# schmeing/ReSeq

Measured on AMD Instinct MI355X. Metric: simulated read-pairs/sec (2x150 bp), higher is better.
Workload: dtype f64

## Files before the change

### reseq_amd/csrc/rsq_host.cpp

```cpp
#include <stdio.h>
#include "rsq_host.h"
#include "rsq_textio.h"

#include <errno.h>
#include <fcntl.h>
#include <string.h>
#include <sys/mman.h>
#include <sys/stat.h>
#include <unistd.h>
#include <zlib.h>

#include <algorithm>
#include <array>
#include <atomic>
#include <chrono>
#include <exception>
#include <memory>
#include <mutex>

#include <fstream>
#include <thread>

#include "rsq_core.h"

namespace rsq {

Options &options() {
    static Options o;
    return o;
}
namespace {
struct OptionEntry {
    const char *name;
    int64_t Options::*field;
};
const OptionEntry kOptionTable[] = {
    {"fill_mode", &Options::fill_mode},         {"image_tiles", &Options::image_tiles},     {"rate_rows", &Options::rate_rows},
    {"no_indel_skip", &Options::no_indel_skip}, {"force_exact", &Options::force_exact},     {"base_call_word", &Options::base_call_word},     {"min_quality_quads", &Options::min_quality_quads},
    {"trace_plan", &Options::trace_plan},       {"trace_prepare", &Options::trace_prepare},
    {"bias_window", &Options::bias_window},     {"window_chunks", &Options::window_chunks}, {"serial_fasta", &Options::serial_fasta},   {"trace_load", &Options::trace_load},
    {"chain_chunk", &Options::chain_chunk},     {"chain_warmup", &Options::chain_warmup},
    {"serial_parse", &Options::serial_parse},   {"parse_stretch", &Options::parse_stretch}, {"mapped_parses", &Options::mapped_parses},
    {"fasta_stretch", &Options::fasta_stretch}, {"overlap", &Options::overlap}, {"specialize", &Options::specialize}, {"job_write_direct", &Options::job_write_direct},             {"job_chunk_bytes", &Options::job_chunk_bytes}, {"host_gzip", &Options::host_gzip}, {"fill_waves", &Options::fill_waves}, {"fasta_no_stage", &Options::fasta_no_stage},
    {"hiprtc_by_name", &Options::hiprtc_by_name}, {"gzip_route", &Options::gzip_route},       {"gzip_stretch", &Options::gzip_stretch},
    {"sieve_lds", &Options::sieve_lds},         {"sieve_lds_bytes", &Options::sieve_lds_bytes}, {"sieve_tracks_mb", &Options::sieve_tracks_mb},
    {"wide_rows", &Options::wide_rows},
    {"stats_chunk", &Options::stats_chunk},     {"stats_slab", &Options::stats_slab},       {"stats_groups", &Options::stats_groups},   {"stats_form", &Options::stats_form},
};
}
bool set_option(const char *name, int64_t value) {
    for (const OptionEntry &e : kOptionTable)
        if (0 == strcmp(name, e.name)) {
            options().*(e.field) = value;
            return true;
        }
    return false;
}
bool get_option(const char *name, int64_t *value) {
    for (const OptionEntry &e : kOptionTable)
        if (0 == strcmp(name, e.name)) {
            *value = options().*(e.field);
            return true;
        }
    return false;
}
const char *option_names() {
    static const std::string names = [] {
        std::string s;
        for (const OptionEntry &e : kOptionTable) s += (s.empty() ? "" : " ") + std::string(e.name);
        return s;
    }();
    return names.c_str();
}

static size_t pad8(size_t n) { return (8 - (n & 7)) & 7; }

Container::Container(const std::string &path) {
    std::ifstream f(path, std::ios::binary | std::ios::ate);
    if (!f) throw Error("cannot open profile '" + path + "'");
    std::streamsize sz = f.tellg();
    f.seekg(0);
    buf_.resize((size_t)sz);
    if (!f.read(reinterpret_cast<char *>(buf_.data()), sz)) throw Error("cannot read profile '" + path + "'");
    if (buf_.size() < 16 || memcmp(buf_.data(), "RSQPROF1", 8) != 0) throw Error("'" + path + "' is not an RSQP profile container");
    uint32_t version, n;
    memcpy(&version, &buf_[8], 4);
    memcpy(&n, &buf_[12], 4);
    if (version != 1) throw Error("unsupported RSQP version");
    static const size_t kSize[7] = {1, 2, 4, 8, 4, 8, 8};
    size_t pos = 16;
    for (uint32_t i = 0; i < n; ++i) {
        if (pos + 4 > buf_.size()) throw Error("truncated RSQP container");
        uint16_t ln;
        memcpy(&ln, &buf_[pos], 2);
        std::string name(reinterpret_cast<const char *>(&buf_[pos + 2]), ln);
        Array a;
        a.dtype = buf_[pos + 2 + ln];
        int ndim = buf_[pos + 3 + ln];
// ... 1206 lines not shown
```

### reseq_amd/csrc/rsq_host.h

```cpp
#pragma once
#include <stdint.h>

#include <map>
#include <stdexcept>
#include <string>
#include <string.h>
#include <vector>

namespace rsq {

struct Error : std::runtime_error {
    using std::runtime_error::runtime_error;
};

struct Options {
    int64_t fill_mode = -1;
    int64_t image_tiles = 0;
    int64_t rate_rows = 0;
    int64_t no_indel_skip = 0;
    int64_t base_call_word = 1;
    int64_t force_exact = 0;
    int64_t min_quality_quads = 0;
    int64_t trace_plan = 0;
    int64_t trace_prepare = 0;
    int64_t bias_window = 0;
    int64_t window_chunks = 0;
    int64_t trace_load = 0;
    int64_t serial_fasta = 0;
    int64_t fasta_stretch = 0;
    int64_t chain_chunk = 0;
    int64_t chain_warmup = -1;
    int64_t serial_parse = 0;
    int64_t mapped_parses = 0;
    int64_t parse_stretch = 0;
    int64_t job_chunk_bytes = 0;
    int64_t job_write_direct = 0;
    int64_t specialize = 1;
    int64_t fasta_no_stage = 0;
    int64_t fill_waves = 0;
    int64_t host_gzip = 0;
    int64_t gzip_route = -1;
    int64_t gzip_stretch = 0;
    int64_t hiprtc_by_name = 0;
    int64_t sieve_lds = 1;
    int64_t sieve_lds_bytes = 0;
    int64_t sieve_tracks_mb = 4096;
    int64_t wide_rows = 0;
    int64_t overlap = 0;
    int64_t stats_chunk = 0;
    int64_t stats_slab = 0;
    int64_t stats_groups = 0;
    int64_t stats_form = 0;
};
Options &options();
bool set_option(const char *name, int64_t value);
bool get_option(const char *name, int64_t *value);
const char *option_names();

struct Array {
    int dtype = 0;
    std::vector<uint64_t> dims;
    uint64_t count = 0;
    const uint8_t *data = nullptr;
};

class Container {
   public:
    explicit Container(const std::string &path);
    const Array &get(const std::string &name) const;
    bool has(const std::string &name) const { return arrays_.count(name) != 0; }
    template <class T>
    std::vector<T> vec(const std::string &name, int dtype) const {
        const Array &a = get(name);
        if (a.dtype != dtype) throw Error("profile array '" + name + "' has the wrong type");
        const T *p = reinterpret_cast<const T *>(a.data);
        return std::vector<T>(p, p + a.count);
    }
    template <class T>
    T scalar(const std::string &name, int dtype) const {
        return vec<T>(name, dtype).at(0);
    }

   private:
    std::vector<uint8_t> buf_;
    std::map<std::string, Array> arrays_;
};

template <class T>
struct Vect {
    uint64_t from = 0;
    std::vector<T> v;
    uint64_t to() const { return from + v.size(); }
    T operator[](uint64_t i) const { return (i < from || i >= to()) ? T(0) : v[i - from]; }
};

struct HostTable {
    uint32_t nm = 0;
    std::vector<uint32_t> par0;
    uint32_t from[4] = {0, 0, 0, 0}, to[4] = {0, 0, 0, 0};
// ... 139 lines not shown
```

### reseq_amd/csrc/rsq_sieve.h

```cpp
#pragma once
#include "rsq_core.h"
#include "rsq_variants.h"

namespace rsq {

struct SieveSite {
    uint32_t seq, start, L;
    uint64_t word_off;
    const double *thr;
    uint32_t group;
    uint32_t sur_start[3];
    bool have_start;
    uint32_t sub;
    VarStart st;
};

RSQ_HD uint32_t site_c1(const SieveSite &site) { return site.seq | (site.sub << 22); }

struct GapTables {
    const double *q_;
    const uint32_t *seg_end_;
    const double *thr_;
    RSQ_HD double q(uint32_t len) const { return q_[len]; }
    RSQ_HD uint32_t seg_end(uint32_t len) const { return seg_end_[len]; }
    RSQ_HD double thr1(uint32_t len) const { return thr_[2u * len + 1u]; }
};
RSQ_HD GapTables gap_tables(const DevSim &S, const SieveSite &site) {
    return GapTables{S.gap_q + (size_t)site.group * S.insert_to, S.gap_seg_end + (size_t)site.group * S.insert_to, site.thr};
}
template <class T, class F>
RSQ_HD uint32_t sieve_gaps_in(const DevSim &S, const SieveSite &site, const T &tab, F &&on_pass) {
    const uint32_t c1 = site_c1(site);
    uint32_t cur = S.insert_from, k = 0, n = 0;
    while (cur < S.insert_to) {
        const Words w = philox(S.seed, site.start, c1, k++, kDomSieve << 28);
        const uint32_t e = tab.seg_end(cur);
        const double base = (cur == S.insert_from || tab.seg_end(cur - 1u) == cur) ? 1.0 : tab.q(cur - 1u);
        const double target = u53_to_unit(w.w0, w.w1) * base;
        uint32_t lo = cur, hi = e;
        while (lo < hi) {
            const uint32_t mid = (lo + hi) >> 1;
            if (tab.q(mid) <= target) hi = mid;
            else lo = mid + 1u;
        }
        if (lo < e) {
            const double thr1 = tab.thr1(lo);
            on_pass(lo, thr1 + u53_to_unit(w.w2, w.w3) * (1 - thr1));
            ++n;
            cur = lo + 1u;
        } else cur = e;
    }
    return n;
}
template <class F>
// ... 461 lines not shown
        if (at < hit_cap) hits[at] = h;
        intra += (uint32_t)h.cnt0 + h.cnt1;
    }
    if (c < cand_cap) pairs_of[c] = n_here;
}

template <int VM>
__global__ void __launch_bounds__(256) k_sieve_emit(DevSim S, uint32_t block_lo, uint32_t block_hi, const SieveHit *hits, uint32_t n_hits, const uint64_t *cand_off,
                                                   const uint64_t *pair_off, Fragment *frags, FragmentVar *fvars, const SlotInfo *slots, const SieveCand *cands = nullptr,
                                                   const uint32_t *pairs_of = nullptr, const uint32_t *cell_info = nullptr) {
    const uint32_t i = blockIdx.x * blockDim.x + threadIdx.x;
    if (i >= n_hits) return;
    SieveHit h;
    if constexpr (VM == 0) {
        const uint32_t pairs = pairs_of[i];
        if (!pairs) return;
        const SieveCand cand = cands[i];
        const uint32_t info = cell_info[i];
        h.slot = cand.slot;
        h.cand = i;
        h.intra = 0;
        h.len = (uint16_t)cand.len;
        h.cnt0 = (uint16_t)(info & 0xFFFFu);
        h.cnt1 = (uint16_t)(pairs - (info & 0xFFFFu));
        h.strand0 = (uint8_t)((info >> 16) & 1u);
        h.strand1 = (uint8_t)((info >> 17) & 1u);
        h.allele0 = h.allele1 = 0;
    } else h = hits[i];
    SieveSite site;
    uint32_t first_slot;
    const uint32_t block_id = init_site_slot<VM>(S, block_lo, block_hi, h.slot, site, &first_slot, slots);
    const uint64_t base = pair_off[h.cand];
    const uint32_t number_base = (uint32_t)(base - pair_off[cand_off[first_slot]]);
    uint32_t k = h.intra;
    for (uint32_t e = 0; e < 2u; ++e) {
        const uint32_t cnt = e ? h.cnt1 : h.cnt0, strand = e ? h.strand1 : h.strand0, allele = e ? h.allele1 : h.allele0;
        if (!cnt) continue;
        FragmentVar fv{};
        if constexpr (VM == 2) {
            const AlleleCell ac = allele_cell(allele_view(S, site.seq, allele), site.st, site.start, h.len);
            fv.end = ac.end;
            fv.sub = site.sub;
            fv.start_var = site.st.first_variant_id;
            fv.start_var_pos = site.st.start_variant_pos;
            fv.end_var = ac.end_var.first_variant_id;
            fv.end_var_pos = ac.end_var.start_variant_pos;
        }
        for (uint32_t dup = 0; dup < cnt; ++dup, ++k) {
            frags[base + k] = make_fragment(site, h.len, dup, strand, block_id, number_base + k + 1u, allele);
            if constexpr (VM == 2) fvars[base + k] = fv;
        }
    }
}
#endif

}
```

### reseq_amd/csrc/rsq_sim.hip

```cpp
#include <hip/hip_runtime.h>
#include <fcntl.h>
#include <sys/mman.h>
#include <sys/stat.h>
#include <math.h>
#include <string.h>
#include <unistd.h>

#include <algorithm>
#include <atomic>
#include <chrono>
#include <map>
#include <thread>
#include <type_traits>
#include <memory>
#include <string>
#include <utility>
#include <vector>

#include "../../include/reseq_amd.h"
#include "rsq_deflate.h"
#include "rsq_fasta.h"
#include "rsq_chains.h"
#include "rsq_sieve.h"
#include "rsq_scan.h"
// ... 143 lines not shown
        std::vector<std::unique_ptr<DevBuf>> &own = owned[current_scope];
        own.emplace_back(new DevBuf());
        own.back()->reserve(bytes + 8);
        HIP_CHECK(hipMemcpy(own.back()->as<void>(), data, bytes, hipMemcpyHostToDevice));
        return own.back()->as<void>();
    }
    void *put_zeros(size_t bytes) override {
        std::vector<std::unique_ptr<DevBuf>> &own = owned[current_scope];
        own.emplace_back(new DevBuf());
        own.back()->reserve(bytes + 8);
        HIP_CHECK(hipMemset(own.back()->as<void>(), 0, bytes + 8));
        return own.back()->as<void>();
    }
    void write_bytes(void *dst, const void *src, size_t bytes) override { HIP_CHECK(hipMemcpy(dst, src, bytes, hipMemcpyHostToDevice)); }
    void read_bytes(void *dst_host, const void *src, size_t bytes) override { HIP_CHECK(hipMemcpy(dst_host, src, bytes, hipMemcpyDeviceToHost)); }
};

struct MappedFile {
    const char *data = nullptr;
    size_t size = 0;
    explicit MappedFile(const char *path) {
        const int fd = open(path, O_RDONLY);
        if (fd < 0) throw Error(std::string("cannot open ") + path + ": " + strerror(errno));
        struct stat st;
        if (fstat(fd, &st) != 0 || st.st_size <= 0) {
            close(fd);
            throw Error(std::string(path) + " is empty or cannot be examined");
        }
        size = (size_t)st.st_size;
        void *p = mmap(nullptr, size, PROT_READ, MAP_PRIVATE, fd, 0);
        close(fd);
        if (p == MAP_FAILED) throw Error(std::string("cannot map ") + path);
        data = static_cast<const char *>(p);
    }
    ~MappedFile() {
        if (data) munmap(const_cast<char *>(data), size);
    }
    MappedFile(const MappedFile &) = delete;
    MappedFile &operator=(const MappedFile &) = delete;
};

struct rsq_sim : PrepassSim {
    int device = 0;
    DeviceUploader up;
    struct Workspace {
        DevBuf fvars;
        DevBuf slot_table;
        DevBuf counts, offsets, tile_sums, scan_total, frags, raw_seq, raw_qual, raw_ops, raw_meta, sizes, off_r1, off_r2, fill_counters, hits, hit_count, cands, pairs_of, pair_off, templates, rec_flags, rec_index, rec_count;
        DevBuf bin_keys, bin_small, bin_perm, bin_frags, bin_fvars;
        DevBuf fa_counts, fa_first, fa_at, fa_len, fa_id_len, fa_frag_len, fa_seg, fa_codes, fa_summary;
        DevBuf sam_sizes, sam_side, off_sam;
        DevBuf bam_side;
        DevBuf cell_info;
        hipEvent_t text_done = nullptr;
    } ws[2];
    struct JobText {
        std::vector<std::unique_ptr<DevBuf>> chunks[2];
        std::vector<size_t> used[2];
        uint64_t bytes[2] = {0, 0};
        bool complete = false;
        std::vector<unsigned char> packed[2];
        bool is_packed = false;
        bool device_packed = false;
        void clear() {
            complete = false;
            is_packed = false;
            device_packed = false;
            for (auto &p : packed) std::vector<unsigned char>().swap(p);
            for (int f = 0; f < 2; ++f) {
                chunks[f].clear();
                used[f].clear();
                bytes[f] = 0;
            }
        }
    } job;
    DevBuf totals;
    bool gz_dense = false;
    bool gz_keep_code = false, gz_have_code = false;
    DevBuf gz_slots, gz_sizes, gz_at, gz_hist, gz_codes, gz_total;
    Workspace *cur = &ws[0];
    hipStream_t side[2] = {nullptr, nullptr};
    hipEvent_t ev_call = nullptr, ev_fill = nullptr, ev_emit = nullptr;
    std::map<std::string, Timer> timers;
    uint32_t n_cu = 256;
    struct Mailbox {
        struct Sieve {
            uint64_t total, n_cands;
            uint32_t n_hits;
        } sieve[2];
        uint64_t r1_bytes, r2_bytes, truth_bytes;
        uint32_t walk_error, longest_record, truth_longest;
        uint32_t bad_fragment;
        uint64_t text_bytes, fasta_starts;
        uint32_t text_longest;
        struct {
            uint32_t longest, first_bad, stray_text, spare;
        } fasta_summary;
        uint32_t fasta_lead_end, fasta_last_start;
    } *mailbox = nullptr;
    uint64_t format_record_bytes = 480;
    DevBuf longest_record;
    DevBuf sam_totals, sam_longest;
    uint64_t sam_pair_bytes = 1100;
    uint64_t bam_pair_bytes = 700;
    bool truth_variants = false;
    bool truth_alleles = false;
    bool truth_md = false;
    struct BamSorted {
        bool active = false;
        bool open = false;
        uint64_t stream_at = 0;
        uint32_t next_block = 0;
        uint64_t prev_cut = 0;
        BamSortPlan plan{};
        DevBuf stage[2], dir[2];
        int cur = 0;
        uint64_t n_held = 0, held_bytes = 0;
        uint64_t call_pairs = 0;
        uint32_t call_parts = 1;
        uint64_t call_records = 0, call_mapped = 0;
        DevBuf keys[2], idx[2], hist, hist_at, sizes, at, flags, run_of, runs, result, out_of_order, windows, window_first;
        BamIndexState index;
    } bam_sorted;
    uint64_t record_text_bytes = 480;
    struct Depth {
        bool open = false, finished = false;
        DevBuf diff, bad, tile_sums;
        uint64_t words = 0;
        uint32_t bg_seq = 0xFFFFFFFFu, bg_carry = 0;
        uint64_t bg_next = 0;
        DevBuf flags, rank, ends, sizes, offsets;
    } depth;
    struct Stats {
        bool open = false;
        DevBuf counts;
        StatsLayout lay{};
    } stats;
    struct Pileup {
        bool open = false, finished = false;
        uint32_t sets = 1;
        DevBuf planes, bad, tile_sums;
// ... 503 lines not shown
        HIP_CHECK(hipMemcpyAsync(&m.truth_bytes, s.sam_totals.as<uint64_t>() + parts, 8, hipMemcpyDeviceToHost, text_stream));
        HIP_CHECK(hipMemcpyAsync(&m.truth_longest, s.sam_longest.as<uint32_t>(), 4, hipMemcpyDeviceToHost, text_stream));
    }
    m.walk_error = 0;
    if (mapped && s.has_variants) HIP_CHECK(hipMemcpyAsync(&m.walk_error, s.dev.walk_error, 4, hipMemcpyDeviceToHost, text_stream));
    static_assert(offsetof(rsq_sim::Mailbox, r2_bytes) == offsetof(rsq_sim::Mailbox, r1_bytes) + 8, "one copy fills both");
    HIP_CHECK(hipMemcpyAsync(&m.r1_bytes, s.totals.as<uint64_t>() + 2 * parts, 16, hipMemcpyDeviceToHost, text_stream));
    HIP_CHECK(hipMemcpyAsync(&m.longest_record, s.longest_record.as<uint32_t>(), 4, hipMemcpyDeviceToHost, text_stream));
    HIP_CHECK(hipStreamSynchronize(text_stream));
    *call.r1.len = m.r1_bytes;
    *call.r2.len = m.r2_bytes;
    int rc = RSQ_OK;
    if (m.walk_error) {
        HIP_CHECK(hipMemsetAsync(s.dev.walk_error, 0, 4, text_stream));
        HIP_CHECK(hipStreamSynchronize(text_stream));
        g_last_error = kWalkErrorMessage;
        rc = RSQ_EINVAL;
    } else if (*call.r1.len > call.r1.cap || *call.r2.len > call.r2.cap || !call.r1.dst || !call.r2.dst) {
        g_last_error = call.need();
        rc = RSQ_ENOSPC;
    }
    if (call.has_truth() && m.truth_longest) (call.bam() ? s.bam_pair_bytes : s.sam_pair_bytes) = m.truth_longest + 16u;
    if (call.has_truth() && !call.sorted()) {
        const uint64_t bytes = *call.truth.len = m.truth_bytes;
        if (rc == RSQ_ENOSPC || (rc == RSQ_OK && (bytes > call.truth.cap || !call.truth.dst))) {
            g_last_error = call.need() + " of FASTQ text and " + std::to_string(bytes) + (call.bam() ? " of BAM records" : " of SAM text");
            rc = RSQ_ENOSPC;
        }
    }
    if (mapped && (rc == RSQ_OK || rc == RSQ_ENOSPC) && m.longest_record) s.format_record_bytes = m.longest_record + 8u;
    return rc;
}

static int adapter_only_pairs(rsq_sim &s, const PairsCall &call, uint64_t n_pairs, uint64_t adapter_first) {
    HIP_CHECK(hipSetDevice(s.device));
    *call.r1.len = *call.r2.len = 0;
    if (call.has_truth()) *call.truth.len = 0;
    if (!n_pairs) return RSQ_OK;
    reset_call_timers(s);
    s.cur = &s.ws[0];
    begin_call(s, call, 1, call.st);
    Part p{nullptr, nullptr, n_pairs, adapter_first, 0};
    reads_stage(s, p, call.st);
    text_stage(s, call, p, call.st);
    if (call.has_truth()) sam_stage(s, call, p, call.st);
    return finish_call(s, call, 1, false, call.st);
}

struct SieveRun {
    uint32_t block_lo = 0, block_hi = 0;
    uint64_t n_slots = 0, cand_cap = 0, hit_cap = 0, total = 0, n_cands = 0;
    uint32_t n_hits = 0;
    const SlotInfo *slot_table = nullptr;
};
static void sieve_attempt(rsq_sim &s, SieveRun &r, int attempt, rsq_sim::Mailbox::Sieve &mail, hipStream_t st) {
    rsq_sim::Workspace &w = *s.cur;
    const int vm = s.variants_mode;
    if (r.cand_cap >= (1ull << 32)) throw Error("more than 2^32 sieve candidates in one call: use smaller block ranges");
    w.cands.reserve(r.cand_cap * sizeof(SieveCand));
    w.pairs_of.reserve(r.cand_cap * 4 + 16);
    w.pair_off.reserve((r.cand_cap + 1) * 8);
    if (vm) w.hits.reserve(r.hit_cap * sizeof(SieveHit));
    else w.cell_info.reserve(r.cand_cap * 4 + 16);
    HIP_CHECK(hipMemsetAsync(w.hit_count.as<uint32_t>(), 0, 4, st));
    s.timers["sieve"].start(st);
    const uint32_t block_lo = r.block_lo, block_hi = r.block_hi;
    const uint64_t n_slots = r.n_slots, cand_cap = r.cand_cap;
    const dim3 ggrid(cdiv(n_slots, kSieveBlock)), gblock(kSieveBlock);
    const size_t lds_bytes = (size_t)(s.dev.insert_to - s.dev.insert_from) * kSieveLdsPerLength;
    const bool in_lds = s.opt.sieve_lds != 0 && lds_bytes <= (s.opt.sieve_lds_bytes > 0 ? (size_t)s.opt.sieve_lds_bytes : kSieveLdsLimit);
    const dim3 lgrid(cdiv(ggrid.x, kSieveTilesPerGroup));
    const SlotInfo *slot_table = r.slot_table;
    auto gaps = [&](auto vm_tag, auto fill_tag, uint32_t *counts, const uint64_t *cand_off, SieveCand *cands) {
        constexpr int kVm = decltype(vm_tag)::value;
        constexpr bool kFill = decltype(fill_tag)::value;
        if (in_lds)
            hipLaunchKernelGGL((k_sieve_gaps_lds<kVm, kFill>), lgrid, gblock, lds_bytes, st, s.dev, block_lo, block_hi, (uint32_t)n_slots, counts, cand_off, cands, cand_cap, slot_table);
        else
            hipLaunchKernelGGL((k_sieve_gaps<kVm, kFill>), ggrid, gblock, 0, st, s.dev, block_lo, block_hi, (uint32_t)n_slots, counts, cand_off, cands, cand_cap, slot_table);
    };
    using Vm0 = std::integral_constant<int, 0>;
    using Vm2 = std::integral_constant<int, 2>;
    if (!attempt) {
        if (2 == vm) {
            w.slot_table.reserve(n_slots * sizeof(SlotInfo) + 16);
            s.timers["slot_table"].start(st);
            hipLaunchKernelGGL(k_slot_table, dim3(block_hi - block_lo), dim3(256), 0, st, s.dev, block_lo, w.slot_table.as<SlotInfo>());
            s.timers["slot_table"].stop(st);
            slot_table = r.slot_table = w.slot_table.as<SlotInfo>();
        }
        s.timers["sieve_screen"].start(st);
        if (2 == vm) gaps(Vm2{}, std::false_type{}, w.counts.as<uint32_t>(), nullptr, nullptr);
        else gaps(Vm0{}, std::false_type{}, w.counts.as<uint32_t>(), nullptr, nullptr);
        s.timers["sieve_screen"].stop(st);
        exclusive_scan(s, w.counts.as<uint32_t>(), n_slots, w.offsets.as<uint64_t>(), st);
    }
    s.timers[in_lds ? "sieve_gaps_lds" : "sieve_gaps_mem"].mark();
    if (2 == vm) gaps(Vm2{}, std::true_type{}, nullptr, w.offsets.as<uint64_t>(), w.cands.as<SieveCand>());
    else gaps(Vm0{}, std::true_type{}, nullptr, w.offsets.as<uint64_t>(), w.cands.as<SieveCand>());
    const dim3 fgrid(cdiv(cand_cap, kSieveBlock)), fblock(kSieveBlock);
    BiasTracks tracks{nullptr, nullptr, 0, 0};
    if (0 == vm && s.sieve_tracks.hi > s.sieve_tracks.lo) {
        auto global_of_block = [&](uint32_t b) { return s.seq_base_off[s.block_seq[b]] + (uint64_t)(b - s.first_block[s.block_seq[b]]) * kBlockSize; };
        const uint64_t first = global_of_block(block_lo), last = std::min<uint64_t>(s.total_ref_size, global_of_block(block_hi - 1u) + kBlockSize + s.dev.insert_to);
        if (first >= s.sieve_tracks.lo && last <= s.sieve_tracks.hi)
            tracks = BiasTracks{s.sieve_tracks.start_bias.as<double>(), s.sieve_tracks.end_bias.as<double>(), s.sieve_tracks.lo, s.sieve_tracks.hi};
    }
    if (0 == vm) s.timers[tracks.hi > tracks.lo ? "sieve_tracks" : "sieve_tracks_off"].mark();
#define RSQ_FINISH(VM, CAP)                                                                                                                                   \
    hipLaunchKernelGGL((k_sieve_finish<VM, CAP>), fgrid, fblock, 0, st, s.dev, block_lo, block_hi, (uint32_t)n_slots, w.offsets.as<uint64_t>(), w.cands.as<SieveCand>(),  \
                       cand_cap, w.pairs_of.as<uint32_t>(), w.hits.as<SieveHit>(), (uint32_t)std::min<uint64_t>(r.hit_cap, 0xFFFFFFFFull), w.hit_count.as<uint32_t>(), slot_table, \
                       w.cell_info.as<uint32_t>(), tracks)
    if (2 == vm && s.num_alleles <= 8) RSQ_FINISH(2, 8);
    else if (2 == vm) RSQ_FINISH(2, kMaxDevAlleles);
    else if (1 == vm) RSQ_FINISH(1, 8);
    else RSQ_FINISH(0, 1);
#undef RSQ_FINISH
    s.timers["sieve"].stop(st);
    HIP_CHECK(hipGetLastError());
    exclusive_scan(s, w.pairs_of.as<uint32_t>(), cand_cap, w.pair_off.as<uint64_t>(), st);
    HIP_CHECK(hipMemcpyAsync(&mail.total, w.pair_off.as<uint64_t>() + cand_cap, 8, hipMemcpyDeviceToHost, st));
    HIP_CHECK(hipMemcpyAsync(&mail.n_hits, w.hit_count.as<uint32_t>(), 4, hipMemcpyDeviceToHost, st));
    HIP_CHECK(hipMemcpyAsync(&mail.n_cands, w.offsets.as<uint64_t>() + n_slots, 8, hipMemcpyDeviceToHost, st));
}
static void sieve_launch(rsq_sim &s, SieveRun &r, uint32_t block_lo, uint32_t block_hi, rsq_sim::Mailbox::Sieve &mail, hipStream_t st) {
    rsq_sim::Workspace &w = *s.cur;
    const int vm = s.variants_mode;
    r = SieveRun{};
    r.block_lo = block_lo;
    r.block_hi = block_hi;
    r.n_slots = (uint64_t)(block_hi - block_lo) * kBlockSize;
    if (2 == vm && block_hi > block_lo) {
        uint32_t ptr[2];
        HIP_CHECK(hipMemcpy(&ptr[0], s.dev.block_extra_ptr + block_lo, 4, hipMemcpyDeviceToHost));
        HIP_CHECK(hipMemcpy(&ptr[1], s.dev.block_extra_ptr + block_hi, 4, hipMemcpyDeviceToHost));
        r.n_slots += ptr[1] - ptr[0];
    }
    if (!r.n_slots) return;
    if (r.n_slots >= (1ull << 32) - kSieveBlock)
        throw Error("block range too large for one call: at most " + std::to_string(((1ull << 32) - kSieveBlock) / kBlockSize - 1) + " blocks");
    w.counts.reserve(r.n_slots * 4 + 16);
    w.offsets.reserve((r.n_slots + 1) * 8);
    w.hit_count.reserve(8);
    const double expected_cands = s.expected_passing * (double)r.n_slots;
    r.cand_cap = std::max<uint64_t>(w.cands.bytes() / sizeof(SieveCand), (uint64_t)(expected_cands + 6.0 * sqrt(expected_cands + 1.0)) + 65536);
    r.hit_cap = std::max<uint64_t>(w.hits.bytes() / sizeof(SieveHit), 0 == vm ? r.cand_cap : r.cand_cap + r.cand_cap / 4);
    sieve_attempt(s, r, 0, mail, st);
}
static void sieve_collect(rsq_sim &s, SieveRun &r, rsq_sim::Mailbox::Sieve &mail, hipStream_t st) {
    for (int attempt = 0;; ++attempt) {
        HIP_CHECK(hipStreamSynchronize(st));
        r.total = mail.total;
        r.n_hits = mail.n_hits;
        r.n_cands = mail.n_cands;
        if (r.n_cands <= r.cand_cap && r.n_hits <= r.hit_cap) return;
        if (attempt >= 2) throw Error("sieve lists overflowed three times");
        const double grow = r.n_cands > r.cand_cap ? (double)r.n_cands / (double)r.cand_cap : 1.0;
        if (r.n_hits > r.hit_cap || grow > 1.0) r.hit_cap = std::max<uint64_t>(r.hit_cap, (uint64_t)((double)r.n_hits * grow * 1.25) + 65536);
        r.cand_cap = std::max(r.cand_cap, r.n_cands + 65536);
        sieve_attempt(s, r, attempt + 1, mail, st);
    }
}
static void sieve_emit(rsq_sim &s, const SieveRun &r, hipStream_t st) {
    rsq_sim::Workspace &w = *s.cur;
    w.frags.reserve(r.total * sizeof(Fragment) + 16);
    s.timers["sieve_emit"].start(st);
    if (2 == s.variants_mode) {
        w.fvars.reserve(r.total * sizeof(FragmentVar) + 16);
        hipLaunchKernelGGL(k_sieve_emit<2>, dim3(cdiv(r.n_hits, 256)), dim3(256), 0, st, s.dev, r.block_lo, r.block_hi, w.hits.as<SieveHit>(), r.n_hits, w.offsets.as<uint64_t>(),
                           w.pair_off.as<uint64_t>(), w.frags.as<Fragment>(), w.fvars.as<FragmentVar>(), w.slot_table.as<SlotInfo>());
    } else if (1 == s.variants_mode)
        hipLaunchKernelGGL(k_sieve_emit<1>, dim3(cdiv(r.n_hits, 256)), dim3(256), 0, st, s.dev, r.block_lo, r.block_hi, w.hits.as<SieveHit>(), r.n_hits, w.offsets.as<uint64_t>(),
                           w.pair_off.as<uint64_t>(), w.frags.as<Fragment>(), (FragmentVar *)nullptr, (const SlotInfo *)nullptr);
    else
        hipLaunchKernelGGL(k_sieve_emit<0>, dim3(cdiv(r.n_cands, 256)), dim3(256), 0, st, s.dev, r.block_lo, r.block_hi, (const SieveHit *)nullptr, (uint32_t)r.n_cands,
                           w.offsets.as<uint64_t>(), w.pair_off.as<uint64_t>(), w.frags.as<Fragment>(), (FragmentVar *)nullptr, (const SlotInfo *)nullptr, w.cands.as<SieveCand>(),
                           w.pairs_of.as<uint32_t>(), w.cell_info.as<uint32_t>());
    s.timers["sieve_emit"].stop(st);
    HIP_CHECK(hipGetLastError());
}

static uint32_t pairs_parts(const rsq_sim &s, uint32_t n_blocks) {
    const int64_t opt = s.opt.overlap;
    if (s.keeps_part()) return 1u;
    return opt > 0 ? (uint32_t)std::min<int64_t>(opt, std::max<uint32_t>(n_blocks, 1u)) : 1u;
}
static int check_block_range(const rsq_sim &s, uint32_t block_lo, uint32_t block_hi) {
    if (!s.prepared || !s.has_ref) {
        g_last_error = "rsq_sim_prepare with a reference must run before rsq_sim_pairs";
        return RSQ_ESTATE;
    }
    if (block_lo < 1 || block_hi > s.total_blocks + 1 || block_lo > block_hi) {
        g_last_error = "block range outside [1, total_blocks]";
        return RSQ_EINVAL;
    }
    if (block_lo < block_hi && (block_lo < s.prepared_lo || block_hi > s.prepared_hi)) {
        g_last_error = "blocks [" + std::to_string(block_lo) + ", " + std::to_string(block_hi) + ") lie outside the range the sharded pre-pass prepared on this simulator, [" +
                       std::to_string(s.prepared_lo) + ", " + std::to_string(s.prepared_hi) + ")";
        return RSQ_ESTATE;
    }
    return RSQ_OK;
}
static int sim_pairs(rsq_sim &s, const PairsCall &call, uint32_t block_lo, uint32_t block_hi, uint64_t *n_pairs) {
    if (const int rc = check_block_range(s, block_lo, block_hi)) return rc;
    HIP_CHECK(hipSetDevice(s.device));
    *n_pairs = 0;
    *call.r1.len = *call.r2.len = 0;
    if (call.has_truth()) *call.truth.len = 0;
    s.kept.have = false;
    if (block_lo == block_hi) return RSQ_OK;
    reset_call_timers(s);
    const uint32_t parts = pairs_parts(s, block_hi - block_lo);
    const hipStream_t st = call.st, s_reads = st, s_sieve = parts > 1 ? s.side[0] : st, s_text = parts > 1 ? s.side[1] : st;
    if (parts > 1) {
        HIP_CHECK(hipEventRecord(s.ev_call, st));
        HIP_CHECK(hipStreamWaitEvent(s_sieve, s.ev_call, 0));
        HIP_CHECK(hipStreamWaitEvent(s_text, s.ev_call, 0));
    }
    begin_call(s, call, parts, s_text);
    struct Abort {
        bool armed = true;
        ~Abort() {
            if (armed) (void)hipDeviceSynchronize();
        }
    } abort_guard;
    auto part_range = [&](uint32_t k) {
// ... 2687 lines not shown
```

Before: 268.1 million.

## Fuse sieve gap screening and cell evaluation into one tiled LDS kernel

Adds a fused k_sieve_tiles kernel for variant-free runs with LDS gap tables. Each tile keeps its passing candidates in shared memory, scans them in-block and writes compact hits with per-tile pair counts. A small scan over tiles and a dedicated emit kernel replace the global candidate list, offsets scan and separate finish pass. The aim is to cut global traffic and kernel launches. It falls back to the split path when a tile overflows its LDS stash, and the extra LDS use may lower occupancy.

```diff
diff --git a/reseq_amd/csrc/rsq_host.cpp b/reseq_amd/csrc/rsq_host.cpp
--- a/reseq_amd/csrc/rsq_host.cpp
+++ b/reseq_amd/csrc/rsq_host.cpp
@@ -44,6 +44,7 @@
     {"fasta_stretch", &Options::fasta_stretch}, {"overlap", &Options::overlap}, {"specialize", &Options::specialize}, {"job_write_direct", &Options::job_write_direct},             {"job_chunk_bytes", &Options::job_chunk_bytes}, {"host_gzip", &Options::host_gzip}, {"fill_waves", &Options::fill_waves}, {"fasta_no_stage", &Options::fasta_no_stage},
     {"hiprtc_by_name", &Options::hiprtc_by_name}, {"gzip_route", &Options::gzip_route},       {"gzip_stretch", &Options::gzip_stretch},
     {"sieve_lds", &Options::sieve_lds},         {"sieve_lds_bytes", &Options::sieve_lds_bytes}, {"sieve_tracks_mb", &Options::sieve_tracks_mb},
+    {"sieve_split", &Options::sieve_split},     {"sieve_tile_stash", &Options::sieve_tile_stash}, {"sieve_tile_cap", &Options::sieve_tile_cap},
     {"wide_rows", &Options::wide_rows},
     {"stats_chunk", &Options::stats_chunk},     {"stats_slab", &Options::stats_slab},       {"stats_groups", &Options::stats_groups},   {"stats_form", &Options::stats_form},
 };
diff --git a/reseq_amd/csrc/rsq_host.h b/reseq_amd/csrc/rsq_host.h
--- a/reseq_amd/csrc/rsq_host.h
+++ b/reseq_amd/csrc/rsq_host.h
@@ -45,6 +45,9 @@
     int64_t sieve_lds = 1;
     int64_t sieve_lds_bytes = 0;
     int64_t sieve_tracks_mb = 4096;
+    int64_t sieve_split = 0;
+    int64_t sieve_tile_stash = 0;
+    int64_t sieve_tile_cap = 0;
     int64_t wide_rows = 0;
     int64_t overlap = 0;
     int64_t stats_chunk = 0;
diff --git a/reseq_amd/csrc/rsq_sieve.h b/reseq_amd/csrc/rsq_sieve.h
--- a/reseq_amd/csrc/rsq_sieve.h
+++ b/reseq_amd/csrc/rsq_sieve.h
@@ -1,5 +1,6 @@
 #pragma once
 #include "rsq_core.h"
+#include "rsq_scan.h"
 #include "rsq_variants.h"
 
 namespace rsq {
@@ -567,6 +568,251 @@
         }
     }
 }
+
+struct SieveTileHit {
+    uint32_t slot, prefix;
+    uint16_t len, cnt0, cnt1;
+    uint8_t strand0, strand1;
+};
+struct SieveTileLds {
+    uint32_t n_len, stash, extra_cap;
+    RSQ_HD uint32_t cells() const { return stash * kSieveBlockLanes + extra_cap; }
+    RSQ_HD size_t q() const { return 0; }
+    RSQ_HD size_t thr1() const { return 8u * (size_t)n_len; }
+    RSQ_HD size_t cell() const { return 16u * (size_t)n_len; }
+    RSQ_HD size_t seg_end() const { return cell() + 8u * (size_t)cells(); }
+    RSQ_HD size_t words() const { return seg_end() + 4u * (size_t)n_len; }
+    RSQ_HD size_t len() const { return words() + 4u * kWords; }
+    RSQ_HD size_t extra_at() const { return len() + 2u * (size_t)cells(); }
+    RSQ_HD size_t off() const { return extra_at() + 2u * (size_t)extra_cap; }
+    RSQ_HD size_t bytes() const { return off() + 2u * kSieveBlockLanes; }
+    static constexpr uint32_t kSieveBlockLanes = 256, kWords = 16;
+    static constexpr uint32_t kWaveSum = 0, kExtras = 8, kHitBase = 9, kCursor = 10;
+};
+constexpr uint32_t kSieveTileStash = 8;
+constexpr uint32_t kSieveTileCapMax = 65535;
+constexpr size_t kSieveTileLdsAim = 40u << 10;
+
+__device__ __forceinline__ uint64_t sieve_tile_scan(uint64_t v, uint32_t *s_wave, uint64_t &total) {
+    const uint32_t lane = threadIdx.x & 63u, wave = threadIdx.x >> 6;
+    uint64_t incl = v;
+    for (uint32_t d = 1; d < 64u; d <<= 1) {
+        const uint64_t t = scan_shfl_up(incl, d);
+        if (lane >= d) incl += t;
+    }
+    if (63u == lane) {
+        s_wave[2u * wave] = (uint32_t)incl;
+        s_wave[2u * wave + 1u] = (uint32_t)(incl >> 32);
+    }
+    __syncthreads();
+    uint64_t front = 0;
+    total = 0;
+    for (uint32_t w = 0; w < kSieveBlock / 64u; ++w) {
+        const uint64_t sum = (uint64_t)s_wave[2u * w] | ((uint64_t)s_wave[2u * w + 1u] << 32);
+        if (w < wave) front += sum;
+        total += sum;
+    }
+    __syncthreads();
+    return front + incl - v;
+}
+
+template <bool TRACKS>
+__global__ void __launch_bounds__(kSieveBlock) k_sieve_tiles(DevSim S, uint32_t block_lo, uint32_t block_hi, uint32_t n_slots, SieveTileLds lay, uint32_t cap, BiasTracks tracks,
+                                                             uint32_t *tile_pairs, uint32_t *boundary_prefix, SieveTileHit *hits, uint32_t hit_cap, uint32_t *hit_count,
+                                                             uint32_t *overflow) {
+    extern __shared__ double s_gap_tables[];
+    unsigned char *s_raw = reinterpret_cast<unsigned char *>(s_gap_tables);
+    const uint32_t from = S.insert_from, n_len = lay.n_len, R = lay.stash, n_cells = lay.cells();
+    double *s_q = reinterpret_cast<double *>(s_raw + lay.q()), *s_thr1 = reinterpret_cast<double *>(s_raw + lay.thr1());
+    uint64_t *s_cell = reinterpret_cast<uint64_t *>(s_raw + lay.cell());
+    uint32_t *s_seg_end = reinterpret_cast<uint32_t *>(s_raw + lay.seg_end()), *s_word = reinterpret_cast<uint32_t *>(s_raw + lay.words());
+    uint16_t *s_len = reinterpret_cast<uint16_t *>(s_raw + lay.len()), *s_extra_at = reinterpret_cast<uint16_t *>(s_raw + lay.extra_at());
+    uint16_t *s_off = reinterpret_cast<uint16_t *>(s_raw + lay.off());
+    const GapTablesLds lds{s_q, s_thr1, s_seg_end, from};
+    const uint32_t tid = threadIdx.x;
+    const uint32_t n_tiles = (n_slots + kSieveBlock - 1u) / kSieveBlock;
+    const uint32_t tile_lo = blockIdx.x * kSieveTilesPerGroup, tile_hi = tile_lo + kSieveTilesPerGroup < n_tiles ? tile_lo + kSieveTilesPerGroup : n_tiles;
+    uint32_t staged = 0xFFFFFFFFu;
+    auto locate = [&](uint32_t i, uint32_t n_extras, uint32_t &lane_of) {
+        uint32_t lo = 0, hi = kSieveBlock;
+        while (hi - lo > 1u) {
+            const uint32_t mid = (lo + hi) >> 1;
+            if (s_off[mid] <= i) lo = mid;
+            else hi = mid;
+        }
+        lane_of = lo;
+        const uint32_t pass = i - s_off[lo];
+        if (pass < R) return pass * kSieveBlock + lo;
+        for (uint32_t j = 0; j < n_extras; ++j)
+            if (s_extra_at[j] == i) return R * kSieveBlock + j;
+        return n_cells;
+    };
+    for (uint32_t tile = tile_lo; tile < tile_hi; ++tile) {
+        SieveSite first;
+        init_site_slot<0, false>(S, block_lo, block_hi, tile * kSieveBlock, first);
+        if (first.group != staged) {
+            const GapTables mem = gap_tables(S, first);
+            for (uint32_t i = tid; i < n_len; i += kSieveBlock) {
+                s_q[i] = mem.q(from + i);
+                s_thr1[i] = mem.thr1(from + i);
+                s_seg_end[i] = mem.seg_end(from + i);
+            }
+            staged = first.group;
+        }
+        if (0u == tid) {
+            s_word[SieveTileLds::kExtras] = 0;
+            s_word[SieveTileLds::kCursor] = 0;
+        }
+        __syncthreads();
+        const uint32_t slot = tile * kSieveBlock + tid;
+        SieveSite site;
+        bool live = slot < n_slots;
+        if (live) {
+            init_site_slot<0, false>(S, block_lo, block_hi, slot, site);
+            live = site.start < site.L;
+        }
+        uint32_t count = 0;
+        if (live) {
+            uint32_t n = 0;
+            auto keep = [&](uint32_t len, double probability_chosen) {
+                if (n < R) {
+                    s_cell[n * kSieveBlock + tid] = (uint64_t)__double_as_longlong(probability_chosen);
+                    s_len[n * kSieveBlock + tid] = (uint16_t)len;
+                }
+                ++n;
+            };
+            if (site.group == staged) count = sieve_gaps_in(S, site, lds, keep);
+            else count = sieve_gaps_in(S, site, gap_tables(S, site), keep);
+        }
+        uint64_t total64;
+        const uint32_t my_off = (uint32_t)sieve_tile_scan(count, s_word + SieveTileLds::kWaveSum, total64);
+        const uint32_t total = (uint32_t)total64;
+        const bool fits = total <= cap;
+        uint32_t extra_at = 0;
+        if (fits) {
+            s_off[tid] = (uint16_t)my_off;
+            if (count > R) extra_at = atomicAdd(&s_word[SieveTileLds::kExtras], count - R);
+        }
+        __syncthreads();
+        const uint32_t n_extras = s_word[SieveTileLds::kExtras];
+        const bool good = fits && n_extras <= lay.extra_cap;
+        if (good && n_extras) {
+            if (count > R) {
+                uint32_t n = 0;
+                auto keep = [&](uint32_t len, double probability_chosen) {
+                    if (n >= R) {
+                        const uint32_t j = extra_at + (n - R);
+                        if (j < lay.extra_cap) {
+                            s_cell[R * kSieveBlock + j] = (uint64_t)__double_as_longlong(probability_chosen);
+                            s_len[R * kSieveBlock + j] = (uint16_t)len;
+                            s_extra_at[j] = (uint16_t)(my_off + n);
+                        }
+                    }
+                    ++n;
+                };
+                if (site.group == staged) sieve_gaps_in(S, site, lds, keep);
+                else sieve_gaps_in(S, site, gap_tables(S, site), keep);
+            }
+            __syncthreads();
+        }
+        uint32_t sum_pairs = 0, sum_hits = 0;
+        if (good) {
+            const uint32_t t0 = tile * kSieveBlock, sb = (t0 + kBlockSize - 1u) / kBlockSize * kBlockSize;
+            const bool has_start = sb - t0 < kSieveBlock && sb < n_slots;
+            const uint32_t boundary_at = has_start ? s_off[sb - t0] : 0xFFFFFFFFu;
+            for (uint32_t i0 = 0; i0 < total; i0 += kSieveBlock) {
+                const uint32_t i = i0 + tid;
+                uint32_t n_here = 0, fwd = 0, rev = 0, at = n_cells;
+                if (i < total) {
+                    uint32_t lane_of;
+                    at = locate(i, n_extras, lane_of);
+                    if (at < n_cells) {
+                        const double probability_chosen = __longlong_as_double((long long)s_cell[at]);
+                        const uint32_t len = s_len[at];
+                        SieveSite cs;
+                        init_site_slot<0>(S, block_lo, block_hi, tile * kSieveBlock + lane_of, cs);
+                        uint32_t cnt[2], strand_of[2];
+                        n_here = sieve_cell_with(S, cs, len, probability_chosen, cnt, strand_of, [&](SieveSite &st, uint32_t end, double &start_factor, double &end_factor) {
+                            if constexpr (TRACKS) {
+                                const uint64_t p = S.seq_base_off[st.seq] + st.start, p_end = S.seq_base_off[st.seq] + end - 1u;
+                                start_factor = tracks.start_bias[p - tracks.lo];
+                                end_factor = tracks.end_bias[p_end - tracks.lo];
+                            } else surrounding_factors(S, st, end, start_factor, end_factor);
+                        });
+                        const bool single_reverse = n_here && 1u == strand_of[0];
+                        fwd = n_here ? (single_reverse ? 0u : cnt[0]) : 0u;
+                        rev = n_here ? (single_reverse ? cnt[0] : cnt[1]) : 0u;
+                    }
+                }
+                uint64_t round_total;
+                const uint64_t before = sieve_tile_scan((uint64_t)n_here | ((uint64_t)(n_here ? 1u : 0u) << 32), s_word + SieveTileLds::kWaveSum, round_total);
+                const uint32_t prefix = sum_pairs + (uint32_t)before;
+                if (at < n_cells) s_cell[at] = (uint64_t)prefix | ((uint64_t)(fwd & 0xFFFFu) << 32) | ((uint64_t)(rev & 0xFFFFu) << 48);
+                if (i < total && i == boundary_at) boundary_prefix[tile] = prefix;
+                sum_pairs += (uint32_t)round_total;
+                sum_hits += (uint32_t)(round_total >> 32);
+            }
+            if (0u == tid) {
+                tile_pairs[tile] = sum_pairs;
+                if (!has_start) boundary_prefix[tile] = 0;
+                else if (boundary_at >= total) boundary_prefix[tile] = sum_pairs;
+                if (sum_hits) s_word[SieveTileLds::kHitBase] = atomicAdd(hit_count, sum_hits);
+            }
+        } else if (0u == tid) {
+            tile_pairs[tile] = 0;
+            boundary_prefix[tile] = 0;
+            atomicOr(overflow, 1u);
+        }
+        __syncthreads();
+        if (good && sum_hits) {
+            const uint32_t hit_base = s_word[SieveTileLds::kHitBase];
+            for (uint32_t i0 = 0; i0 < total; i0 += kSieveBlock) {
+                const uint32_t i = i0 + tid;
+                uint32_t lane_of = 0, at = n_cells;
+                if (i < total) at = locate(i, n_extras, lane_of);
+                const uint64_t cell = at < n_cells ? s_cell[at] : 0u;
+                const uint32_t fwd = (uint32_t)(cell >> 32) & 0xFFFFu, rev = (uint32_t)(cell >> 48);
+                const bool hit = 0u != (fwd | rev);
+                const uint64_t mask = __ballot(hit);
+                if (!mask) continue;
+                const uint32_t lane = tid & 63u, leader = (uint32_t)__ffsll((long long)mask) - 1u;
+                uint32_t wave_at = 0;
+                if (lane == leader) wave_at = atomicAdd(&s_word[SieveTileLds::kCursor], (uint32_t)__popcll(mask));
+                wave_at = (uint32_t)__shfl((int)wave_at, (int)leader, 64);
+                const uint64_t place = (uint64_t)hit_base + wave_at + (uint32_t)__popcll(mask & ((1ull << lane) - 1ull));
+                if (hit && place < hit_cap) {
+                    SieveTileHit h;
+                    h.slot = tile * kSieveBlock + lane_of;
+                    h.prefix = (uint32_t)cell;
+                    h.len = s_len[at];
+                    h.cnt0 = (uint16_t)fwd;
+                    h.cnt1 = (uint16_t)rev;
+                    h.strand0 = 0;
+                    h.strand1 = 1;
+                    hits[place] = h;
+                }
+            }
+        }
+        __syncthreads();
+    }
+}
+
+__global__ void __launch_bounds__(256) k_sieve_emit_tiles(DevSim S, uint32_t block_lo, uint32_t block_hi, const SieveTileHit *hits, uint32_t n_hits, const uint64_t *tile_off,
+                                                         const uint32_t *boundary_prefix, Fragment *frags) {
+    const uint32_t i = blockIdx.x * blockDim.x + threadIdx.x;
+    if (i >= n_hits) return;
+    const SieveTileHit h = hits[i];
+    SieveSite site;
+    uint32_t first_slot;
+    const uint32_t block_id = init_site_slot<0>(S, block_lo, block_hi, h.slot, site, &first_slot);
+    const uint64_t base = tile_off[h.slot / kSieveBlock] + h.prefix;
+    const uint32_t number_base = (uint32_t)(base - (tile_off[first_slot / kSieveBlock] + boundary_prefix[first_slot / kSieveBlock]));
+    uint32_t k = 0;
+    for (uint32_t e = 0; e < 2u; ++e) {
+        const uint32_t cnt = e ? h.cnt1 : h.cnt0, strand = e ? h.strand1 : h.strand0;
+        for (uint32_t dup = 0; dup < cnt; ++dup, ++k) frags[base + k] = make_fragment(site, h.len, dup, strand, block_id, number_base + k + 1u);
+    }
+}
 #endif
 
 }
diff --git a/reseq_amd/csrc/rsq_sim.hip b/reseq_amd/csrc/rsq_sim.hip
--- a/reseq_amd/csrc/rsq_sim.hip
+++ b/reseq_amd/csrc/rsq_sim.hip
@@ -219,6 +219,7 @@
         DevBuf sam_sizes, sam_side, off_sam;
         DevBuf bam_side;
         DevBuf cell_info;
+        DevBuf tile_pairs, tile_off, boundary_prefix, tile_hits, tile_overflow;
         hipEvent_t text_done = nullptr;
     } ws[2];
     struct JobText {
@@ -254,6 +255,7 @@
         struct Sieve {
             uint64_t total, n_cands;
             uint32_t n_hits;
+            uint32_t tile_overflow;
         } sieve[2];
         uint64_t r1_bytes, r2_bytes, truth_bytes;
         uint32_t walk_error, longest_record, truth_longest;
@@ -863,8 +865,55 @@
     uint64_t n_slots = 0, cand_cap = 0, hit_cap = 0, total = 0, n_cands = 0;
     uint32_t n_hits = 0;
     const SlotInfo *slot_table = nullptr;
+    bool tiles = false;
+    SieveTileLds tile_lds{};
+    uint32_t tile_cap = 0;
 };
+static BiasTracks sieve_bias_tracks(rsq_sim &s, uint32_t block_lo, uint32_t block_hi) {
+    BiasTracks tracks{nullptr, nullptr, 0, 0};
+    if (0 == s.variants_mode && s.sieve_tracks.hi > s.sieve_tracks.lo) {
+        auto global_of_block = [&](uint32_t b) { return s.seq_base_off[s.block_seq[b]] + (uint64_t)(b - s.first_block[s.block_seq[b]]) * kBlockSize; };
+        const uint64_t first = global_of_block(block_lo), last = std::min<uint64_t>(s.total_ref_size, global_of_block(block_hi - 1u) + kBlockSize + s.dev.insert_to);
+        if (first >= s.sieve_tracks.lo && last <= s.sieve_tracks.hi)
+            tracks = BiasTracks{s.sieve_tracks.start_bias.as<double>(), s.sieve_tracks.end_bias.as<double>(), s.sieve_tracks.lo, s.sieve_tracks.hi};
+    }
+    if (0 == s.variants_mode) s.timers[tracks.hi > tracks.lo ? "sieve_tracks" : "sieve_tracks_off"].mark();
+    return tracks;
+}
+static bool sieve_tables_in_lds(const rsq_sim &s) {
+    const size_t lds_bytes = (size_t)(s.dev.insert_to - s.dev.insert_from) * kSieveLdsPerLength;
+    return s.opt.sieve_lds != 0 && lds_bytes <= (s.opt.sieve_lds_bytes > 0 ? (size_t)s.opt.sieve_lds_bytes : kSieveLdsLimit);
+}
+static void sieve_tiles_attempt(rsq_sim &s, SieveRun &r, rsq_sim::Mailbox::Sieve &mail, hipStream_t st) {
+    rsq_sim::Workspace &w = *s.cur;
+    const uint32_t n_tiles = cdiv(r.n_slots, kSieveBlock);
+    w.tile_pairs.reserve((size_t)n_tiles * 4 + 16);
+    w.tile_off.reserve(((size_t)n_tiles + 1) * 8);
+    w.boundary_prefix.reserve((size_t)n_tiles * 4 + 16);
+    w.tile_hits.reserve(r.hit_cap * sizeof(SieveTileHit));
+    w.tile_overflow.reserve(8);
+    HIP_CHECK(hipMemsetAsync(w.hit_count.as<uint32_t>(), 0, 4, st));
+    HIP_CHECK(hipMemsetAsync(w.tile_overflow.as<uint32_t>(), 0, 4, st));
+    s.timers["sieve"].start(st);
+    s.timers["sieve_gaps_lds"].mark();
+    s.timers["sieve_fused"].mark();
+    const BiasTracks tracks = sieve_bias_tracks(s, r.block_lo, r.block_hi);
+    s.timers["sieve_screen"].start(st);
+    hipLaunchKernelGGL(tracks.hi > tracks.lo ? k_sieve_tiles<true> : k_sieve_tiles<false>, dim3(cdiv(n_tiles, kSieveTilesPerGroup)), dim3(kSieveBlock), r.tile_lds.bytes(), st, s.dev,
+                       r.block_lo, r.block_hi, (uint32_t)r.n_slots, r.tile_lds, r.tile_cap, tracks, w.tile_pairs.as<uint32_t>(), w.boundary_prefix.as<uint32_t>(),
+                       w.tile_hits.as<SieveTileHit>(), (uint32_t)std::min<uint64_t>(r.hit_cap, 0xFFFFFFFFull), w.hit_count.as<uint32_t>(), w.tile_overflow.as<uint32_t>());
+    s.timers["sieve_screen"].stop(st);
+    s.timers["sieve"].stop(st);
+    HIP_CHECK(hipGetLastError());
+    s.timers["scan"].start(st);
+    exclusive_scan(s, w.tile_pairs.as<uint32_t>(), n_tiles, w.tile_off.as<uint64_t>(), st);
+    s.timers["scan"].stop(st);
+    HIP_CHECK(hipMemcpyAsync(&mail.total, w.tile_off.as<uint64_t>() + n_tiles, 8, hipMemcpyDeviceToHost, st));
+    HIP_CHECK(hipMemcpyAsync(&mail.n_hits, w.hit_count.as<uint32_t>(), 4, hipMemcpyDeviceToHost, st));
+    HIP_CHECK(hipMemcpyAsync(&mail.tile_overflow, w.tile_overflow.as<uint32_t>(), 4, hipMemcpyDeviceToHost, st));
+}
 static void sieve_attempt(rsq_sim &s, SieveRun &r, int attempt, rsq_sim::Mailbox::Sieve &mail, hipStream_t st) {
+    if (r.tiles) return sieve_tiles_attempt(s, r, mail, st);
     rsq_sim::Workspace &w = *s.cur;
     const int vm = s.variants_mode;
     if (r.cand_cap >= (1ull << 32)) throw Error("more than 2^32 sieve candidates in one call: use smaller block ranges");
@@ -879,7 +928,7 @@
     const uint64_t n_slots = r.n_slots, cand_cap = r.cand_cap;
     const dim3 ggrid(cdiv(n_slots, kSieveBlock)), gblock(kSieveBlock);
     const size_t lds_bytes = (size_t)(s.dev.insert_to - s.dev.insert_from) * kSieveLdsPerLength;
-    const bool in_lds = s.opt.sieve_lds != 0 && lds_bytes <= (s.opt.sieve_lds_bytes > 0 ? (size_t)s.opt.sieve_lds_bytes : kSieveLdsLimit);
+    const bool in_lds = sieve_tables_in_lds(s);
     const dim3 lgrid(cdiv(ggrid.x, kSieveTilesPerGroup));
     const SlotInfo *slot_table = r.slot_table;
     auto gaps = [&](auto vm_tag, auto fill_tag, uint32_t *counts, const uint64_t *cand_off, SieveCand *cands) {
@@ -910,14 +959,7 @@
     if (2 == vm) gaps(Vm2{}, std::true_type{}, nullptr, w.offsets.as<uint64_t>(), w.cands.as<SieveCand>());
     else gaps(Vm0{}, std::true_type{}, nullptr, w.offsets.as<uint64_t>(), w.cands.as<SieveCand>());
     const dim3 fgrid(cdiv(cand_cap, kSieveBlock)), fblock(kSieveBlock);
-    BiasTracks tracks{nullptr, nullptr, 0, 0};
-    if (0 == vm && s.sieve_tracks.hi > s.sieve_tracks.lo) {
-        auto global_of_block = [&](uint32_t b) { return s.seq_base_off[s.block_seq[b]] + (uint64_t)(b - s.first_block[s.block_seq[b]]) * kBlockSize; };
-        const uint64_t first = global_of_block(block_lo), last = std::min<uint64_t>(s.total_ref_size, global_of_block(block_hi - 1u) + kBlockSize + s.dev.insert_to);
-        if (first >= s.sieve_tracks.lo && last <= s.sieve_tracks.hi)
-            tracks = BiasTracks{s.sieve_tracks.start_bias.as<double>(), s.sieve_tracks.end_bias.as<double>(), s.sieve_tracks.lo, s.sieve_tracks.hi};
-    }
-    if (0 == vm) s.timers[tracks.hi > tracks.lo ? "sieve_tracks" : "sieve_tracks_off"].mark();
+    const BiasTracks tracks = sieve_bias_tracks(s, block_lo, block_hi);
 #define RSQ_FINISH(VM, CAP)                                                                                                                                   \
     hipLaunchKernelGGL((k_sieve_finish<VM, CAP>), fgrid, fblock, 0, st, s.dev, block_lo, block_hi, (uint32_t)n_slots, w.offsets.as<uint64_t>(), w.cands.as<SieveCand>(),  \
                        cand_cap, w.pairs_of.as<uint32_t>(), w.hits.as<SieveHit>(), (uint32_t)std::min<uint64_t>(r.hit_cap, 0xFFFFFFFFull), w.hit_count.as<uint32_t>(), slot_table, \
@@ -956,13 +998,43 @@
     const double expected_cands = s.expected_passing * (double)r.n_slots;
     r.cand_cap = std::max<uint64_t>(w.cands.bytes() / sizeof(SieveCand), (uint64_t)(expected_cands + 6.0 * sqrt(expected_cands + 1.0)) + 65536);
     r.hit_cap = std::max<uint64_t>(w.hits.bytes() / sizeof(SieveHit), 0 == vm ? r.cand_cap : r.cand_cap + r.cand_cap / 4);
+    if (0 == vm && !s.opt.sieve_split && sieve_tables_in_lds(s)) {
+        const double m = s.expected_passing;
+        const uint32_t rows = s.opt.sieve_tile_stash > 0 ? (uint32_t)std::min<int64_t>(s.opt.sieve_tile_stash, 64)
+                                                         : (uint32_t)std::min(64.0, std::max<double>(kSieveTileStash, ceil(m + 4.5 * sqrt(m))));
+        SieveTileLds lay{s.dev.insert_to - s.dev.insert_from, rows, 0u};
+        const size_t fixed = lay.bytes();
+        lay.extra_cap = (uint32_t)std::min<size_t>(4096, std::max<size_t>(16, fixed < kSieveTileLdsAim ? (kSieveTileLdsAim - fixed) / 12u : 0));
+        if (lay.bytes() <= (s.opt.sieve_tile_stash > 0 ? kSieveLdsLimit : kSieveTileLdsAim)) {
+            r.tiles = true;
+            r.tile_lds = lay;
+            r.tile_cap = (uint32_t)std::min<int64_t>(s.opt.sieve_tile_cap > 0 ? s.opt.sieve_tile_cap : kSieveTileCapMax, kSieveTileCapMax);
+            r.hit_cap = std::max<uint64_t>(w.tile_hits.bytes() / sizeof(SieveTileHit), r.cand_cap);
+        }
+    }
     sieve_attempt(s, r, 0, mail, st);
 }
 static void sieve_collect(rsq_sim &s, SieveRun &r, rsq_sim::Mailbox::Sieve &mail, hipStream_t st) {
-    for (int attempt = 0;; ++attempt) {
+    int attempt = 0;
+    for (;; ++attempt) {
         HIP_CHECK(hipStreamSynchronize(st));
         r.total = mail.total;
         r.n_hits = mail.n_hits;
+        if (r.tiles) {
+            if (mail.tile_overflow) {
+                s.timers["sieve_fused_overflow"].mark();
+                r.tiles = false;
+                r.hit_cap = std::max<uint64_t>(s.cur->hits.bytes() / sizeof(SieveHit), r.cand_cap);
+                sieve_attempt(s, r, 0, mail, st);
+                attempt = -1;
+                continue;
+            }
+            if (r.n_hits <= r.hit_cap) return;
+            if (attempt >= 2) throw Error("sieve lists overflowed three times");
+            r.hit_cap = (uint64_t)r.n_hits + 65536;
+            sieve_attempt(s, r, attempt + 1, mail, st);
+            continue;
+        }
         r.n_cands = mail.n_cands;
         if (r.n_cands <= r.cand_cap && r.n_hits <= r.hit_cap) return;
         if (attempt >= 2) throw Error("sieve lists overflowed three times");
@@ -983,6 +1055,9 @@
     } else if (1 == s.variants_mode)
         hipLaunchKernelGGL(k_sieve_emit<1>, dim3(cdiv(r.n_hits, 256)), dim3(256), 0, st, s.dev, r.block_lo, r.block_hi, w.hits.as<SieveHit>(), r.n_hits, w.offsets.as<uint64_t>(),
                            w.pair_off.as<uint64_t>(), w.frags.as<Fragment>(), (FragmentVar *)nullptr, (const SlotInfo *)nullptr);
+    else if (r.tiles)
+        hipLaunchKernelGGL(k_sieve_emit_tiles, dim3(cdiv(r.n_hits, 256)), dim3(256), 0, st, s.dev, r.block_lo, r.block_hi, w.tile_hits.as<SieveTileHit>(), r.n_hits, w.tile_off.as<uint64_t>(),
+                           w.boundary_prefix.as<uint32_t>(), w.frags.as<Fragment>());
     else
         hipLaunchKernelGGL(k_sieve_emit<0>, dim3(cdiv(r.n_cands, 256)), dim3(256), 0, st, s.dev, r.block_lo, r.block_hi, (const SieveHit *)nullptr, (uint32_t)r.n_cands,
                            w.offsets.as<uint64_t>(), w.pair_off.as<uint64_t>(), w.frags.as<Fragment>(), (FragmentVar *)nullptr, (const SlotInfo *)nullptr, w.cands.as<SieveCand>(),
```

Result: no change. 267.2 million (-0.3%).
